# KrishnaswamyLab/MELD

Hardware: AMD Instinct MI355X
Metric: cells/sec through MELD.fit_transform (kNN+Chebyshev) (higher is better)
Workload: dtype f64

## Files before the change

### include/meld_hip.h

```cpp
#ifndef MELD_HIP_H
#define MELD_HIP_H

#include <stddef.h>
#include <stdint.h>

#ifdef __cplusplus
extern "C" {
#endif

#define MELD_OK 0
#define MELD_ERR_INVALID (-1)
#define MELD_ERR_UNSUPPORTED (-2)
#define MELD_ERR_HIP (-3)

typedef void* meld_stream_t;

int meld_abi_version(void);
const char* meld_last_error(void);
int meld_device_count(void);


int meld_knn_padded_dim(int d);
int meld_knn_tile_refs(void);
int meld_knn_block_queries(void);
int meld_knn_row_capacity(int ksel);
double meld_knn_error_coef(int d);

int meld_col_sums_f64(const double* X, int64_t N, int d, double* sums, meld_stream_t stream);
size_t meld_col_stats_temp_bytes(int d);
int meld_col_stats_f64(const double* X, int64_t N, int d, double* sums, double* mins, double* maxs, void* temp, size_t temp_bytes,
                       meld_stream_t stream);

int meld_knn_prepare_refs(const double* X, int64_t N, int d, const double* mean, int KP, float* Rt,
                          float* norm2, float* norm2_max, meld_stream_t stream);
int meld_knn_prepare_queries(const double* X, int64_t N, int d, const double* mean, int KP,
                             int64_t q_begin, int64_t q_count, float* Q, meld_stream_t stream);

int meld_knn_topk(const float* Q, const float* Rt, int64_t n_ref, int KP, int64_t q_count, int ksel,
                  int32_t* cand_idx, float* cand_d2, int32_t* cand_cnt, meld_stream_t stream);

int meld_knn16_kblocks(int d);
int meld_knn16_tile_refs(void);
int meld_knn16_split_dims(int d);
int meld_frame_max_dims(void);
int meld_cov_sample_f64(const double* X, int64_t N, int d, const double* mean, int64_t stride, double* cov, meld_stream_t stream);
int meld_rotate_rows_f64(const double* X, int64_t N, int d, const double* mean, const double* At, double* out, meld_stream_t stream);
int meld_knn16_block_queries(void);
int meld_knn16_row_capacity(int ksel);
double meld_knn16_error_coef(int nprod, int d);
double meld_knn16_error_coef_const(int nprod, int d);
double meld_knn16_error_coef_lin(int nprod);
size_t meld_knn16_tile_bytes(int d);
size_t meld_knn16_query_bytes(int d);
int meld_knn16_prepare(const double* X, int64_t N, int d, const double* mean, int64_t q_begin,
                       int64_t q_count, void* Rt16, void* Q16, float* Qn, float* norm2, float* norm2_max,
                       float* scale_info, meld_stream_t stream);
int meld_knn16_prepare_scaled(const double* X, int64_t N, int d, const double* mean, const double* col_min, const double* col_max,
                              int64_t q_begin, int64_t q_count, void* Rt16, void* Q16, float* Qn, float* norm2, float* norm2_max,
                              float* scale_info, meld_stream_t stream);
size_t meld_knn16_bounds_bytes(int64_t n_ref, int64_t q_count);
size_t meld_knn16_bounds_temp_bytes(int64_t n_ref, int d, int64_t q_count);
int meld_knn16_bounds(const double* X, int64_t N, int d, const double* mean, const float* scale_info,
                      const float* norm2_max, const void* Rt16, int64_t q_begin, int64_t q_count,
                      const float* thr_seed, const float* q_norm2 ,
                      int nprod, void* temp, void* lb2, meld_stream_t stream);
int meld_knn16_tile_spheres(const double* X, int64_t N, int d, const double* mean, const float* scale_info, void* temp,
                            int64_t tile_begin, int64_t tile_count, meld_stream_t stream);
int meld_knn16_sphere_layout(int64_t n_ref, int d, int64_t* rows, int64_t* row_bytes);
int meld_knn16_bounds_from_spheres(const double* X, int64_t N, int d, const double* mean, const float* scale_info,
                      const float* norm2_max, const void* Rt16, int64_t q_begin, int64_t q_count,
                      const float* thr_seed, const float* q_norm2 ,
                      int nprod, void* temp, void* lb2, meld_stream_t stream);
int meld_knn16_prepare_cross(const double* X, int64_t n_refs, int64_t n_total, int d, const double* mean, int64_t q_begin,
                             int64_t q_count, void* Rt16, void* Q16, float* Qn, float* norm2, float* norm2_max,
                             float* scale_info, meld_stream_t stream);
int meld_knn16_prepare_rows(const double* X, int64_t N, int d, const double* mean, const float* scale_info,
                            int64_t q_begin, const int32_t* rows, int64_t n_rows, void* Q16, float* Qn,
                            meld_stream_t stream);
int meld_knn16_research_thresholds(const int32_t* rows, int64_t n_rows, int64_t q_begin, const int32_t* cand_cnt,
// ... 235 lines not shown
```

### meld_amd/_lib.py

```python
from __future__ import annotations

from ._options import is_set, opt

import ctypes as C
import os

_HERE = os.path.dirname(os.path.abspath(__file__))
LIB_NAME = "libmeld_hip.so"
LIB_PATH = os.path.join(_HERE, LIB_NAME)

_i32, _i64, _f64, _sz, _ptr = C.c_int, C.c_int64, C.c_double, C.c_size_t, C.c_void_p

SIGNATURES = {
    "meld_abi_version": (_i32, []),
    "meld_last_error": (C.c_char_p, []),
    "meld_device_count": (_i32, []),
    "meld_knn_padded_dim": (_i32, [_i32]),
    "meld_knn_tile_refs": (_i32, []),
    "meld_knn_block_queries": (_i32, []),
    "meld_knn_row_capacity": (_i32, [_i32]),
    "meld_col_sums_f64": (_i32, [_ptr, _i64, _i32, _ptr, _ptr]),
    "meld_col_stats_temp_bytes": (_sz, [_i32]),
    "meld_col_stats_f64": (_i32, [_ptr, _i64, _i32, _ptr, _ptr, _ptr, _ptr, _sz, _ptr]),
    "meld_knn_prepare_refs": (_i32, [_ptr, _i64, _i32, _ptr, _i32, _ptr, _ptr, _ptr, _ptr]),
# ... 72 lines not shown
        [_ptr, _ptr, _ptr, _ptr, _i64, _i64, _i32, _ptr, _i64, _ptr, _ptr, _ptr, _f64, _f64, _f64, _f64, _ptr, _ptr],
    ),
    "meld_lanczos_steps": (_i32, [_ptr, _ptr, _ptr, _ptr, _i64, _i64, _ptr, _ptr, _ptr, _ptr, _ptr, _ptr, _i32, _i32, _ptr, _ptr]),
    "meld_lanczos_spmv": (_i32, [_ptr, _ptr, _ptr, _ptr, _i64, _i64, _ptr, _i64, _ptr, _ptr, _ptr, _ptr, _ptr]),
    "meld_lanczos_alpha": (_i32, [_ptr, _ptr, _ptr, _ptr, _i32, _ptr]),
    "meld_lanczos_axpy": (_i32, [_ptr, _ptr, _i64, _ptr, _ptr, _ptr]),
    "meld_lanczos_beta": (_i32, [_ptr, _ptr, _ptr, _ptr, _i32, _ptr]),
    "meld_lanczos_fold": (_i32, [_ptr, _ptr, _ptr, _ptr, _i32, _ptr]),
    "meld_lanczos_axpy3": (_i32, [_ptr, _ptr, _ptr, _i64, _ptr, _ptr, _ptr]),
    "meld_pt_geometry": (_i32, [_ptr, _ptr, _ptr, _ptr]),
    "meld_pt_num_blocks": (_i32, [_i64]),
    "meld_pt_seg_len": (_i64, [_i32]),
    "meld_pt_debug_ablate": (_i32, [_i32]),
    "meld_pt_debug_stamps": (_i32, [_ptr]),
    "meld_pt_stream_len": (_i64, [_i64, _i32]),
    "meld_pt_desc_len": (_i64, [_i32]),
    "meld_pt_build": (_i32, [_ptr, _ptr, _ptr, _i64, _i64, _i64, _i32, _ptr, _ptr, _ptr, _ptr]),
    "meld_cheby_step_wide": (_i32, [_ptr, _ptr, _ptr, _ptr, _i64, _i32, _ptr, _i64, _ptr, _ptr, _f64, _f64, _f64, _ptr]),
    "meld_pt_cheby_step": (_i32, [_ptr, _ptr, _ptr, _i64, _i32, _ptr, _i64, _ptr, _ptr, _ptr, _f64, _f64, _f64, _f64, _ptr, _ptr]),
    "meld_pt_cheby_run": (_i32, [_ptr, _ptr, _ptr, _i64, _i32, _ptr, _ptr, _ptr, _ptr, _i32, _f64, _f64, _ptr, _ptr]),
    "meld_pt_lanczos_steps": (_i32, [_ptr, _ptr, _ptr, _i64, _ptr, _ptr, _ptr, _ptr, _ptr, _ptr, _i32, _i32, _ptr, _ptr, _ptr]),
    "meld_pt_lanczos_spmv": (_i32, [_ptr, _ptr, _ptr, _i64, _ptr, _i64, _ptr, _ptr, _ptr, _ptr, _ptr]),
    "meld_kmeans_max_blocks": (_i32, []),
    "meld_kmeans_assign": (_i32, [_ptr, _i64, _i32, _ptr, _i32, _ptr, _ptr, _ptr, _ptr, _i32, _ptr]),
    "meld_scale_f64": (_i32, [_ptr, _f64, _ptr, _i64, _ptr]),
    "meld_axpby_f64": (_i32, [_f64, _ptr, _f64, _ptr, _i64, _ptr, _ptr]),
    "meld_normalize_rows_l1": (_i32, [_ptr, _ptr, _i64, _i32, _ptr]),
    "meld_assign_nearest": (_i32, [_ptr, _i64, _i32, _ptr, _i32, _ptr, _ptr, _ptr, _ptr]),
    "meld_chain_order": (_i32, [_ptr, _i64, _i32, _i32, _ptr, _ptr]),
    "meld_gather_rows_f64": (_i32, [_ptr, _ptr, _i64, _i32, _ptr, _ptr]),
    "meld_frame_max_dims": (_i32, []),
    "meld_cov_sample_f64": (_i32, [_ptr, _i64, _i32, _ptr, _i64, _ptr, _ptr]),
    "meld_rotate_rows_f64": (_i32, [_ptr, _i64, _i32, _ptr, _ptr, _ptr, _ptr]),
    "meld_argsort_u32_temp_bytes": (_sz, [_i64]),
    "meld_argsort_u32": (_i32, [_ptr, _i64, _i32, _ptr, _ptr, _ptr, _sz, _ptr]),
    "meld_order_starts": (_i32, [_ptr, _i64, _i32, _ptr, _ptr]),
    "meld_order_pick_centroids": (_i32, [_ptr, _i64, _i32, _ptr, _ptr, _i32, _i32, _ptr, _ptr]),
    "meld_order_update_keys": (_i32, [_ptr, _ptr, _ptr, _i64, _i32, _ptr]),
    "meld_rccl_available": (_i32, []),
    "meld_rccl_unique_id": (_i32, [_ptr]),
    "meld_rccl_comm_create": (_i32, [_ptr, _i32, _i32, _ptr]),
    "meld_rccl_comm_destroy": (_i32, [_ptr]),
    "meld_rccl_all_gather": (_i32, [_ptr, _ptr, _ptr, _sz, _ptr]),
    "meld_rccl_all_reduce_sum_f64": (_i32, [_ptr, _ptr, _sz, _ptr]),
    "meld_cheby_run_sharded": (_i32, [_ptr, _ptr, _ptr, _ptr, _ptr, _ptr, _i64, _i64, _i64, _i64, _i32, _ptr, _ptr, _ptr, _ptr, _i32, _f64, _f64, _ptr, _ptr]),
    "meld_lanczos_steps_sharded": (_i32, [_ptr, _ptr, _ptr, _ptr, _ptr, _ptr, _i64, _i64, _i64, _i64, _ptr, _ptr, _ptr, _ptr, _ptr, _ptr, _ptr, _i32, _i32, _ptr]),
    "meld_factorize_max_groups": (_i32, []),
    "meld_factorize_max_words": (_i32, []),
    "meld_factorize_temp_bytes": (_sz, [_i64]),
    "meld_factorize_labels": (_i32, [_ptr, _i64, _i32, _ptr, _sz, _ptr, _ptr]),
    "meld_factorize_codes": (_i32, [_ptr, _i64, _ptr, _ptr, _ptr]),
    "meld_indicator_signal": (_i32, [_ptr, _ptr, _ptr, _i64, _i64, _i32, _ptr, _ptr]),
    "meld_scatter_rows_f64": (_i32, [_ptr, _ptr, _i64, _i32, _ptr, _ptr]),
}



class PtLayout(C.Structure):

    _fields_ = [("blk_row", _ptr), ("blk_ntile", _ptr), ("blk_ndist", _ptr), ("seg", _ptr), ("list_cols", _ptr),
                ("pval", _ptr), ("pidx", _ptr), ("nb", C.c_int32), ("pval32", _ptr), ("stream_len", C.c_int64), ("cdesc", _ptr)]


_lib = None


# ... 33 lines not shown
```

### meld_amd/csrc/common.hpp

```cpp
#pragma once
#include <hip/hip_runtime.h>
#include <stdint.h>
#include <stdio.h>
#include <stdlib.h>
#include <string.h>

#include "../../include/meld_hip.h"

namespace meld {

char* err_buf();
void set_err(const char* fmt, ...);

static inline hipStream_t S(meld_stream_t s) { return reinterpret_cast<hipStream_t>(s); }

constexpr int WAVE = 64;

#define MELD_CHECK_ARG(cond, ...)        \
  do {                                   \
    if (!(cond)) {                       \
      meld::set_err(__VA_ARGS__);        \
      return MELD_ERR_INVALID;           \
    }                                    \
  } while (0)

#define MELD_LAUNCH_CHECK(name)                                               \
  do {                                                                        \
    hipError_t e__ = hipGetLastError();                                       \
    if (e__ != hipSuccess) {                                                  \
      meld::set_err("%s: launch failed: %s", name, hipGetErrorString(e__));   \
      return MELD_ERR_HIP;                                                    \
    }                                                                         \
  } while (0)

#define MELD_HIP_CALL(expr)                                                   \
  do {                                                                        \
    hipError_t e__ = (expr);                                                  \
    if (e__ != hipSuccess) {                                                  \
      meld::set_err("%s failed: %s", #expr, hipGetErrorString(e__));          \
      return MELD_ERR_HIP;                                                    \
    }                                                                         \
  } while (0)

__device__ __forceinline__ double wave_sum(double v) {
#pragma unroll
  for (int off = 32; off > 0; off >>= 1) v += __shfl_xor(v, off, 64);
  return v;
}

__device__ __forceinline__ int lane_id() { return threadIdx.x & 63; }

static inline int64_t ceil_div(int64_t a, int64_t b) { return (a + b - 1) / b; }

static inline const char* meld_dev_getenv(const char* name) {
  const char* dev = getenv("MELD_DEV");
  return (dev && dev[0] == '1' && dev[1] == 0) ? getenv(name) : nullptr;
}

struct PtLanczos {
  const double* nrm2_prev;
  double* nrm2_zero;
  const double* state_prev;
  double* state_cur;
  double* betas;
  int it;
  const int* stop;
};

int pt_step(const meld_pt_layout_t* L, const int64_t* rowptr, const double* dw, int p, const double* x_full,
            int64_t x_row_offset, const double* z, double* y, double* r, double alpha, double beta, double gamma,
            double coef, double* dots, const double* coef_dev, hipStream_t st, double coef_x = 0.0, const PtLanczos* lz = nullptr);

}
```

### meld_amd/csrc/frame.hip

```cpp
#include "common.hpp"

namespace meld {

constexpr int FR_ROWS = 64;
constexpr int FR_DMAX = 64;

__global__ __launch_bounds__(256) void cov_sample_kernel(const double* __restrict__ X, int64_t n_s, int64_t stride, int d,
                                                         const double* __restrict__ mean, double* __restrict__ out) {
  __shared__ double sx[FR_ROWS][FR_DMAX + 1];
  const int tid = threadIdx.x;
  const int64_t s0 = (int64_t)blockIdx.x * FR_ROWS;
  const int cnt = (int)min((int64_t)FR_ROWS, n_s - s0);
  for (int u = tid; u < FR_ROWS * d; u += 256) {
    const int r = u / d, k = u - r * d;
    sx[r][k] = r < cnt ? X[(s0 + r) * stride * d + k] - mean[k] : 0.0;
  }
  __syncthreads();
  for (int p = tid; p < d * d; p += 256) {
    const int i = p / d, j = p - i * d;
    if (j < i) continue;
    double acc = 0.0;
    for (int r = 0; r < FR_ROWS; ++r) acc = fma(sx[r][i], sx[r][j], acc);
    atomicAdd(out + p, acc);
  }
}

typedef double f64x8 __attribute__((ext_vector_type(8)));
typedef const __attribute__((address_space(4))) f64x8* const_f64x8_ptr;
constexpr int FR_LD = FR_DMAX + 1;
constexpr int FR_NQ = FR_ROWS * FR_DMAX / 256;
constexpr int FR_CPG = FR_DMAX / 4;
__global__ __launch_bounds__(256) void rotate_rows_kernel(const double* __restrict__ X, int64_t N, int d, const double* __restrict__ mean,
                                                          const double* __restrict__ At, double* __restrict__ out, int64_t tiles_per_wg) {
  __shared__ double sx[FR_ROWS][FR_LD];
  const int tid = threadIdx.x, lane = tid & 63;
  const int w = __builtin_amdgcn_readfirstlane(tid >> 6);
  const int cpg = (d + 3) >> 2;
  const int j0 = w * cpg;
  const int k8n = (d + 7) >> 3;
  const double mk = (lane < d) ? mean[lane] : 0.0;
  const int64_t n_tiles = (N + FR_ROWS - 1) / FR_ROWS;
  const int64_t t_begin = (int64_t)blockIdx.x * tiles_per_wg, t_end = min(n_tiles, t_begin + tiles_per_wg);
// ... 29 lines not shown
        const_f64x8_ptr arow[4];
#pragma unroll
        for (int i = 0; i < 4; ++i)
          arow[i] = (const_f64x8_ptr)(uintptr_t)(At + (size_t)min(j0 + c4 + i, d - 1) * FR_DMAX);
#pragma unroll
        for (int k8 = 0; k8 < FR_DMAX / 8; ++k8) {
          if (k8 < k8n) {
            f64x8 av[4];
#pragma unroll
            for (int i = 0; i < 4; ++i) av[i] = arow[i][k8];
#pragma unroll
            for (int e = 0; e < 8; ++e)
#pragma unroll
              for (int i = 0; i < 4; ++i) acc[i] = fma(xr[8 * k8 + e], av[i][e], acc[i]);
          }
        }
      }
#pragma unroll
      for (int i = 0; i < 4; ++i) res[c4 + i] = acc[i];
    }
    __syncthreads();
#pragma unroll
    for (int c = 0; c < FR_CPG; ++c)
      if (c < cpg && j0 + c < d) sx[lane][j0 + c] = res[c];
    __syncthreads();
#pragma unroll
    for (int q = 0; q < FR_NQ; ++q) {
      const int u = tid + 256 * q, rr = u >> 6, k = u & 63;
      if (rr < cnt && k < d) out[(row0 + rr) * d + k] = sx[rr][k];
    }
  }
}

}

using namespace meld;

extern "C" int meld_frame_max_dims(void) { return FR_DMAX; }

extern "C" int meld_cov_sample_f64(const double* X, int64_t N, int d, const double* mean, int64_t stride, double* cov, meld_stream_t stream) {
  MELD_CHECK_ARG(X && mean && cov && N > 0 && d > 0 && d <= FR_DMAX && stride >= 1, "meld_cov_sample_f64: bad arguments (d <= %d)", FR_DMAX);
  const int64_t n_s = (N + stride - 1) / stride;
  hipLaunchKernelGGL(cov_sample_kernel, dim3((unsigned)ceil_div(n_s, FR_ROWS)), dim3(256), 0, S(stream), X, n_s, stride, d, mean, cov);
  MELD_LAUNCH_CHECK("cov_sample_kernel");
  return MELD_OK;
}

extern "C" int meld_rotate_rows_f64(const double* X, int64_t N, int d, const double* mean, const double* At, double* out, meld_stream_t stream) {
  MELD_CHECK_ARG(X && mean && At && out && N > 0 && d > 0 && d <= FR_DMAX && X != out, "meld_rotate_rows_f64: bad arguments (d <= %d)", FR_DMAX);
  const int64_t tiles = ceil_div(N, FR_ROWS);
  const int64_t per = ceil_div(tiles, (int64_t)1024);
  hipLaunchKernelGGL(rotate_rows_kernel, dim3((unsigned)ceil_div(tiles, per)), dim3(256), 0, S(stream), X, N, d, mean, At, out, per);
  MELD_LAUNCH_CHECK("rotate_rows_kernel");
  return MELD_OK;
}
```

### meld_amd/csrc/knn.hip

```cpp
#include "common.hpp"

#include <algorithm>

namespace meld {

constexpr int KNN_TS = 64;
constexpr int KNN_BQ = 128;
constexpr int KNN_THREADS = 256;
constexpr int KNN_SLACK = 64;
constexpr int KNN_CAPMAX = 192;
constexpr float KNN_BIG = 1.0e30f;

typedef float f32x16 __attribute__((ext_vector_type(16)));

__device__ __forceinline__ float ld_l2_f(const float* p) {
  return __hip_atomic_load(p, __ATOMIC_RELAXED, __HIP_MEMORY_SCOPE_AGENT);
}
__device__ __forceinline__ int ld_l2_i(const int* p) {
  return __hip_atomic_load(p, __ATOMIC_RELAXED, __HIP_MEMORY_SCOPE_AGENT);
}

__device__ float knn_compact_row(int n, int ksel, float* __restrict__ d2row, int* __restrict__ idxrow,
                                 float* sd, int* si, int lane) {
  asm volatile("s_waitcnt vmcnt(0)" ::: "memory");
// ... 256 lines not shown
  float* dst = Q + (size_t)q * KP;
  for (int c = 0; c < KP; ++c)
    dst[c] = (c < d) ? (float)(xrow[c] - mean[c]) : (c == d ? n : (c == d + 1 ? 1.0f : 0.0f));
}

static const int kSupportedKP[] = {8, 12, 16, 24, 32, 40, 52, 64, 80, 104, 128};

}

using namespace meld;

extern "C" int meld_knn_padded_dim(int d) {
  if (d < 1) return MELD_ERR_INVALID;
  for (int kp : kSupportedKP)
    if (d + 2 <= kp) return kp;
  set_err("meld_knn_padded_dim: d=%d exceeds the largest instantiated distance kernel (d <= 126)", d);
  return MELD_ERR_UNSUPPORTED;
}
extern "C" double meld_knn_error_coef(int d) {
  const int kp = meld_knn_padded_dim(d);
  return kp < 0 ? -1.0 : (double)kp * 4.76837158203125e-07;
}
extern "C" int meld_knn_tile_refs(void) { return KNN_TS; }
extern "C" int meld_knn_block_queries(void) { return KNN_BQ; }
extern "C" int meld_knn_row_capacity(int ksel) {
  if (ksel < 1 || ksel > KNN_CAPMAX - KNN_SLACK) {
    set_err("meld_knn_row_capacity: ksel=%d outside [1, %d]", ksel, KNN_CAPMAX - KNN_SLACK);
    return MELD_ERR_UNSUPPORTED;
  }
  return ksel + KNN_SLACK;
}

namespace meld {
constexpr int COL_STATS_GRID = 1024;
__global__ __launch_bounds__(256) void col_stats_kernel(const double* __restrict__ X, int64_t N, int d, double* __restrict__ part) {
  __shared__ double ps[256], pmin[256], pmax[256];
  const int tid = threadIdx.x;
  const int rpp = 256 / d;
  const int c = tid % d;
  const int rl = tid / d;
  double s = 0.0, mn = INFINITY, mx = -INFINITY;
  if (rl < rpp) {
    for (int64_t row = (int64_t)blockIdx.x * rpp + rl; row < N; row += (int64_t)gridDim.x * rpp) {
      const double v = X[row * d + c];
      s += v;
      mn = fmin(mn, v);
      mx = fmax(mx, v);
    }
  }
  ps[tid] = s;
  pmin[tid] = mn;
  pmax[tid] = mx;
  __syncthreads();
  if (tid < d) {
    double ts = 0.0, tmn = INFINITY, tmx = -INFINITY;
    for (int k = 0; k < rpp; ++k) {
      ts += ps[k * d + tid];
      tmn = fmin(tmn, pmin[k * d + tid]);
      tmx = fmax(tmx, pmax[k * d + tid]);
    }
    const size_t g = gridDim.x;
    part[(0 * g + blockIdx.x) * d + tid] = ts;
    part[(1 * g + blockIdx.x) * d + tid] = tmn;
    part[(2 * g + blockIdx.x) * d + tid] = tmx;
  }
}
__global__ __launch_bounds__(256) void col_stats_finish_kernel(const double* __restrict__ part, int grid, int d, double* __restrict__ sums,
                                                               double* __restrict__ mins, double* __restrict__ maxs) {
  __shared__ double ps[256], pmin[256], pmax[256];
  const int c = blockIdx.x, tid = threadIdx.x;
  double ts = 0.0, tmn = INFINITY, tmx = -INFINITY;
  for (int b = tid; b < grid; b += 256) {
    ts += part[((size_t)0 * grid + b) * d + c];
    tmn = fmin(tmn, part[((size_t)1 * grid + b) * d + c]);
    tmx = fmax(tmx, part[((size_t)2 * grid + b) * d + c]);
  }
  ps[tid] = ts;
  pmin[tid] = tmn;
  pmax[tid] = tmx;
  __syncthreads();
  for (int w = 128; w > 0; w >>= 1) {
    if (tid < w) {
      ps[tid] += ps[tid + w];
      pmin[tid] = fmin(pmin[tid], pmin[tid + w]);
      pmax[tid] = fmax(pmax[tid], pmax[tid + w]);
    }
    __syncthreads();
  }
  if (tid == 0) {
    sums[c] = ps[0];
    mins[c] = pmin[0];
    maxs[c] = pmax[0];
  }
}
}
extern "C" size_t meld_col_stats_temp_bytes(int d) { return sizeof(double) * 3 * (size_t)meld::COL_STATS_GRID * (size_t)(d > 0 ? d : 1); }
extern "C" int meld_col_stats_f64(const double* X, int64_t N, int d, double* sums, double* mins, double* maxs, void* temp, size_t temp_bytes,
                                  meld_stream_t stream) {
  using namespace meld;
  MELD_CHECK_ARG(X && sums && mins && maxs && temp && N > 0 && d > 0 && d <= 256, "meld_col_stats_f64: bad arguments (d must be <= 256)");
  MELD_CHECK_ARG(temp_bytes >= meld_col_stats_temp_bytes(d), "meld_col_stats_f64: temp too small");
  const int rpp = 256 / d;
  const int grid = (int)std::min<int64_t>(COL_STATS_GRID, ceil_div(N, rpp));
  hipLaunchKernelGGL(col_stats_kernel, dim3(grid), dim3(256), 0, S(stream), X, N, d, reinterpret_cast<double*>(temp));
  hipLaunchKernelGGL(col_stats_finish_kernel, dim3((unsigned)d), dim3(256), 0, S(stream), reinterpret_cast<const double*>(temp), grid, d,
                     sums, mins, maxs);
  MELD_LAUNCH_CHECK("col_stats_kernel");
  return MELD_OK;
}

extern "C" int meld_col_sums_f64(const double* X, int64_t N, int d, double* sums, meld_stream_t stream) {
  MELD_CHECK_ARG(X && sums && N > 0 && d > 0 && d <= 256, "meld_col_sums_f64: bad arguments (d must be <= 256)");
  MELD_HIP_CALL(hipMemsetAsync(sums, 0, sizeof(double) * d, S(stream)));
  const int rpp = 256 / d;
  int grid = (int)std::min<int64_t>(1024, ceil_div(N, rpp));
  hipLaunchKernelGGL(col_sums_kernel, dim3(grid), dim3(256), 0, S(stream), X, N, d, sums);
  MELD_LAUNCH_CHECK("col_sums_kernel");
  return MELD_OK;
}

extern "C" int meld_knn_prepare_refs(const double* X, int64_t N, int d, const double* mean, int KP, float* Rt,
                                     float* norm2, float* norm2_max, meld_stream_t stream) {
  MELD_CHECK_ARG(X && mean && Rt && norm2 && norm2_max && N > 0, "meld_knn_prepare_refs: null/empty argument");
  MELD_CHECK_ARG(KP == meld_knn_padded_dim(d), "meld_knn_prepare_refs: KP=%d does not match d=%d", KP, d);
  const int64_t n_pad = ceil_div(N, KNN_TS) * KNN_TS;
  hipLaunchKernelGGL(prepare_refs_kernel, dim3((unsigned)ceil_div(n_pad, 256)), dim3(256), 0, S(stream), X, N, d,
// ... 51 lines not shown
```

### meld_amd/graph.py

```python
from __future__ import annotations

from ._options import is_set, opt

import math
import os
import sys
import time

import numpy as np
import torch

from ._lib import check, get_lib, ptr

__all__ = ["DeviceGraph", "build_knn_graph", "default_ksel", "EVENTS", "record_events"]

EVENTS = {"enabled": False, "pairs": []}


def record_events(enabled=True):
    EVENTS["enabled"] = bool(enabled)
    EVENTS["pairs"] = []


class _EventSpan:
# ... 325 lines not shown

            _BLAS_CTL = ThreadpoolController()
        with _BLAS_CTL.limit(limits=1, user_api="blas"):
            return np.linalg.eigh(a, UPLO="U")
    except ImportError:
        return np.linalg.eigh(a, UPLO="U")


def _scan_i32(lib, x, st):
    n = x.shape[0]
    out = torch.empty(n + 1, dtype=torch.int64, device=x.device)
    tb = lib.meld_scan_temp_bytes(n)
    tmp = torch.empty(tb, dtype=torch.uint8, device=x.device)
    check(lib.meld_exclusive_scan_i32_i64(ptr(x), ptr(out), n, ptr(tmp), tb, st), "meld_exclusive_scan_i32_i64")
    return out


class HipOps:

    name = "hip"

    def __init__(self, device=None, search=None, prune=None, nprod=None, spmm=None):
        self.lib = get_lib()
        self.spmm = spmm
        self.nprod = int(opt("MELD_KNN_NPROD", "1")) if nprod is None else int(nprod)
        self.prune = (opt("MELD_KNN_PRUNE", "1") != "0") if prune is None else bool(prune)
        self.radius_cut = opt("MELD_KNN_RADIUS_CUT", "1") != "0"
        self.seed = opt("MELD_KNN_SEED", "1") != "0"
        self.seeded_bounds = opt("MELD_KNN_SEEDED_BOUNDS", "1") != "0"
        self.block_order = opt("MELD_KNN_BLOCK_ORDER", "1") != "0"
        self.step_lists = opt("MELD_KNN_STEP_LISTS", "1") != "0"
        self.rotate = opt("MELD_KNN_ROTATE", "1") != "0"
        self.rotate_min_cells = int(opt("MELD_KNN_ROTATE_MIN", "262144"))
        self.search = search or opt("MELD_KNN_SEARCH", "f16x3")
        if self.search not in ("f16x3", "f32"):
            raise ValueError("unknown search kernel {!r}".format(self.search))
        if not torch.cuda.is_available():
            raise RuntimeError("meld_amd needs a ROCm GPU (MI355X); there is no CPU fallback")
        self.device = torch.device("cuda", torch.cuda.current_device()) if device is None else torch.device(device)

    def col_stats(self, X):
        N, d = int(X.shape[0]), int(X.shape[1])
        out = torch.empty(3, d, dtype=torch.float64, device=X.device)
        tb = self.lib.meld_col_stats_temp_bytes(d)
        tmp = torch.empty(tb, dtype=torch.uint8, device=X.device)
        check(self.lib.meld_col_stats_f64(ptr(X), N, d, ptr(out[0]), ptr(out[1]), ptr(out[2]), ptr(tmp), tb, _stream()), "meld_col_stats_f64")
        return out[0], out[1], out[2]

    def frame_axes_async(self, X, col_stats):
        lib = self.lib
        N, d = int(X.shape[0]), int(X.shape[1])
        if (col_stats is None or opt("MELD_FRAME_ASYNC", "1") == "0" or not self.rotate or not self.prune or not self.step_lists or not self.seed or self.nprod != 1 or self.search != "f16x3"
                or N < max(16384, self.rotate_min_cells) or d > int(lib.meld_frame_max_dims()) or int(lib.meld_knn16_split_dims(d)) <= 0):
            return None
        st = _stream()
        mean = col_stats[0] / N
        cov = torch.zeros(d, d, dtype=torch.float64, device=X.device)
        check(lib.meld_cov_sample_f64(ptr(X), N, d, ptr(mean), max(1, N // 32768), ptr(cov), st), "meld_cov_sample_f64")
        host = torch.empty(d, d, dtype=torch.float64, pin_memory=True)
        host.copy_(cov, non_blocking=True)
        done = torch.cuda.Event()
        done.record()

        def finish(lead):
            done.synchronize()
            evals, evecs = _eigh_one_thread(host.numpy())
            tot = float(evals.sum())
            if not np.isfinite(tot) or tot <= 0.0 or float(evals[-lead:].sum()) < 0.5 * tot:
                return False
            At = np.zeros((d, int(lib.meld_frame_max_dims())))
            At[:, :d] = evecs[:, ::-1].T
            return torch.from_numpy(At).to(X.device, non_blocking=True)

        return finish

    def principal_frame(self, X, mean, lead, comm=None, axes=None):
        lib, st = self.lib, _stream()
        N, d = int(X.shape[0]), int(X.shape[1])
        if axes is not None and (comm is None or getattr(comm, "world", 1) == 1):
            At = axes(lead)
            if At is False:
                return None
            out = torch.empty_like(X)
            check(lib.meld_rotate_rows_f64(ptr(X), N, d, ptr(mean), ptr(At), ptr(out), st), "meld_rotate_rows_f64")
            return out
        wide = d > int(lib.meld_frame_max_dims())
        stride = max(1, N // 32768)
        if wide:
            Xs = X[::stride] - mean
            cov = torch.triu(Xs.T @ Xs)
            del Xs
        else:
            cov = torch.zeros(d, d, dtype=torch.float64, device=X.device)
            check(lib.meld_cov_sample_f64(ptr(X), N, d, ptr(mean), stride, ptr(cov), st), "meld_cov_sample_f64")
        if comm is not None and getattr(comm, "world", 1) > 1:
            if comm.rank != 0:
                cov.zero_()
            comm.all_reduce_sum(cov)
        evals, evecs = _eigh_one_thread(cov.cpu().numpy())
        tot = float(evals.sum())
        if not np.isfinite(tot) or tot <= 0.0 or float(evals[-lead:].sum()) < 0.5 * tot:
            return None
        if wide:
            V = torch.from_numpy(np.ascontiguousarray(evecs[:, ::-1])).to(X.device)
            return torch.addmm(-(mean @ V), X, V)
        At = np.zeros((d, int(lib.meld_frame_max_dims())))
        At[:, :d] = evecs[:, ::-1].T
        At = torch.from_numpy(At).to(X.device)
        out = torch.empty_like(X)
        check(lib.meld_rotate_rows_f64(ptr(X), N, d, ptr(mean), ptr(At), ptr(out), st), "meld_rotate_rows_f64")
        return out

    def directed_kernel_coo(self, X, q_begin, q_count, knn, decay, thresh, ksel, tm=None, force_fallback=False, n_refs=None, assemble=False, comm=None,
                            bw_scale=1.0, bw_fixed=None, col_stats=None, knn_max=None, symm=(0, 0.0), count_rows_ge=None, frame_axes=None):
        lib, st, dev = self.lib, _stream(), X.device
        tm = tm or _Timer(False)
        N, d = int(X.shape[0]), int(X.shape[1])
        cross = n_refs is not None
        NR = int(n_refs) if cross else N
        if cross and not (0 < NR <= q_begin and q_begin + q_count <= N):
            raise ValueError("cross search: the queries must lie behind the n_refs references")
        tm.start()
        col_min = col_max = None
        if col_stats is not None:
            sums, col_min, col_max = col_stats
            mean = sums / N
        elif d <= 256:
            sums, col_min, col_max = self.col_stats(X)
            mean = sums / N
        else:
            mean = X.mean(dim=0)
        norm2 = torch.empty(N, dtype=torch.float32, device=dev)
        nmax = torch.zeros(1, dtype=torch.float32, device=dev)
        X_search, mean_search = X, mean
        search = self.search
        cand_thr, rfac, tiles_done = None, 1.0, None
        used_prune = used_seed = used_seeded_bounds = used_block_order = used_step_lists = used_two_phase = False
        partial_in_search = 0
        if search == "f16x3" and lib.meld_knn16_kblocks(d) < 0:
            search = "wide"
        if cross and search != "f16x3":
            raise NotImplementedError("the search between two point sets runs on the split-fp16 MFMA kernel only (d <= 141)")
        if search == "wide":
            research = None
# ... 16 lines not shown
                    nq = n2[q_begin + q0 : q_begin + q1]
                    best_d = torch.full((q1 - q0, 0), 0.0, dtype=torch.float64, device=dev)
                    best_i = torch.zeros((q1 - q0, 0), dtype=torch.int64, device=dev)
                    for r0 in range(0, N, RC):
                        r1 = min(N, r0 + RC)
                        D = nq[:, None] + n2[None, r0:r1] - 2.0 * (Xq @ Xc[r0:r1].T)
                        ids = torch.arange(r0, r1, device=dev, dtype=torch.int64)[None, :].expand(q1 - q0, -1)
                        D = torch.cat([best_d, D], dim=1)
                        ids = torch.cat([best_i, ids], dim=1)
                        best_d, sel = torch.topk(D, min(kk, D.shape[1]), dim=1, largest=False, sorted=True)
                        best_i = torch.gather(ids, 1, sel)
                    rows = torch.arange(q0, q1, device=dev, dtype=torch.int64)[:, None] * cap + torch.arange(kk, device=dev)[None, :]
                    cand_d2[rows.reshape(-1)] = best_d.clamp_(min=0.0).to(torch.float32).reshape(-1)
                    cand_idx[rows.reshape(-1)] = best_i.to(torch.int32).reshape(-1)
            KP = d
            Q = Rt = None
            del Xc
        elif search == "f16x3":
            nprod = 3 if (self.nprod == 1 and d <= 6) else self.nprod
            KB = lib.meld_knn16_kblocks(d)
            if KB < 0:
                check(KB, "meld_knn16_kblocks")
            TS, BQ = lib.meld_knn16_tile_refs(), lib.meld_knn16_block_queries()
            cap = lib.meld_knn16_row_capacity(ksel)
            if cap < 0:
                check(cap, "meld_knn16_row_capacity")
            err_coef = lib.meld_knn16_error_coef_const(nprod, d)
            err_lin = lib.meld_knn16_error_coef_lin(nprod)
            n_tiles = (NR + TS - 1) // TS
            q_pad = ((q_count + BQ - 1) // BQ) * BQ
            lead = int(lib.meld_knn16_split_dims(d))
            if (self.rotate and lead > 0 and nprod == 1 and not cross and self.prune and self.step_lists and self.seed
                    and N >= max(16384, self.rotate_min_cells) and q_begin % BQ == 0 and bw_fixed is None):
                X_s = self.principal_frame(X, mean, lead, comm, axes=frame_axes)
                if X_s is not None:
                    sums_s, col_min, col_max = self.col_stats(X_s)
                    X_search, mean_search = X_s, sums_s / N
            Rt = torch.empty(n_tiles * lib.meld_knn16_tile_bytes(d), dtype=torch.uint8, device=dev)
            Q = torch.empty(q_pad * lib.meld_knn16_query_bytes(d), dtype=torch.uint8, device=dev)
            Qn = torch.empty(q_pad, dtype=torch.float32, device=dev)
            scale_info = torch.empty(4, dtype=torch.float32, device=dev)
            if cross:
                check(lib.meld_knn16_prepare_cross(ptr(X), NR, N, d, ptr(mean), q_begin, q_count, ptr(Rt), ptr(Q), ptr(Qn), ptr(norm2), ptr(nmax), ptr(scale_info), st), "meld_knn16_prepare_cross")
                norm2[q_begin : q_begin + q_count] = Qn[:q_count]
                nmax = torch.maximum(nmax, Qn[:q_count].max().reshape(1))
            else:
                if col_min is not None:
                    check(lib.meld_knn16_prepare_scaled(ptr(X_search), N, d, ptr(mean_search), ptr(col_min), ptr(col_max), q_begin, q_count, ptr(Rt), ptr(Q), ptr(Qn), ptr(norm2), ptr(nmax), ptr(scale_info), st), "meld_knn16_prepare_scaled")
                else:
                    check(lib.meld_knn16_prepare(ptr(X_search), N, d, ptr(mean_search), q_begin, q_count, ptr(Rt), ptr(Q), ptr(Qn), ptr(norm2), ptr(nmax), ptr(scale_info), st), "meld_knn16_prepare")
            tm.stop("prepare")
            cand_idx = torch.empty(q_pad * cap, dtype=torch.int32, device=dev)
            cand_d2 = torch.empty(q_pad * cap, dtype=torch.float32, device=dev)
            cand_cnt = torch.empty(q_pad, dtype=torch.int32, device=dev)
            if self.radius_cut and knn < ksel:
                cand_thr = torch.full((q_pad,), float("inf"), dtype=torch.float32, device=dev)
                rfac = 1.0 if math.isinf(decay) else float((-math.log(thresh)) ** (1.0 / decay))
                rfac = max(rfac * float(bw_scale), 1.0)
            lb2 = block_order = step_list = step_cnt = None
            tiles_done = torch.zeros(4, dtype=torch.int64, device=dev)
            will_prune = self.prune and q_begin % TS == 0 and N >= 16384 and not cross
            n_blocks = q_pad // BQ
            seeds = None
            knn_cut = knn
            if bw_fixed is not None and cand_thr is not None:
                knn_cut = 0
                rf_real = 1.0 if math.isinf(decay) else float((-math.log(thresh)) ** (1.0 / decay))
                rad = (bw_fixed[q_begin : q_begin + q_count] * float(bw_scale)).clamp_(min=float(np.finfo(float).eps)) * rf_real
                nmx = nmax.to(torch.float64)
# ... 870 lines not shown
```

Measured before the change: 28.06 million.

## Fuse principal-frame rotation with column stats and widen frame to 128 dims

Adds a tiled rotation kernel that computes the rotated rows and, in the same pass, per-column sum, min and max partials, which a shared finish kernel then reduces. This avoids a second full read of the rotated matrix that the separate column-stats pass needed. It also raises the supported frame width from 64 to 128 dims, so the wider case takes the custom rotation path instead of a torch addmm and may be rotated where it was not before. The cost is a more complex kernel with register and LDS tradeoffs that vary with the template width.

```diff
diff --git a/include/meld_hip.h b/include/meld_hip.h
--- a/include/meld_hip.h
+++ b/include/meld_hip.h
@@ -43,8 +43,11 @@
 int meld_knn16_tile_refs(void);
 int meld_knn16_split_dims(int d);
 int meld_frame_max_dims(void);
+int meld_frame_wide_max_dims(void);
 int meld_cov_sample_f64(const double* X, int64_t N, int d, const double* mean, int64_t stride, double* cov, meld_stream_t stream);
 int meld_rotate_rows_f64(const double* X, int64_t N, int d, const double* mean, const double* At, double* out, meld_stream_t stream);
+int meld_rotate_rows_wide_f64(const double* X, int64_t N, int d, const double* mean, const double* At, double* out, double* sums,
+                              double* mins, double* maxs, void* temp, size_t temp_bytes, meld_stream_t stream);
 int meld_knn16_block_queries(void);
 int meld_knn16_row_capacity(int ksel);
 double meld_knn16_error_coef(int nprod, int d);
diff --git a/meld_amd/_lib.py b/meld_amd/_lib.py
--- a/meld_amd/_lib.py
+++ b/meld_amd/_lib.py
@@ -128,6 +128,8 @@
     "meld_frame_max_dims": (_i32, []),
     "meld_cov_sample_f64": (_i32, [_ptr, _i64, _i32, _ptr, _i64, _ptr, _ptr]),
     "meld_rotate_rows_f64": (_i32, [_ptr, _i64, _i32, _ptr, _ptr, _ptr, _ptr]),
+    "meld_frame_wide_max_dims": (_i32, []),
+    "meld_rotate_rows_wide_f64": (_i32, [_ptr, _i64, _i32, _ptr, _ptr, _ptr, _ptr, _ptr, _ptr, _ptr, _sz, _ptr]),
     "meld_argsort_u32_temp_bytes": (_sz, [_i64]),
     "meld_argsort_u32": (_i32, [_ptr, _i64, _i32, _ptr, _ptr, _ptr, _sz, _ptr]),
     "meld_order_starts": (_i32, [_ptr, _i64, _i32, _ptr, _ptr]),
diff --git a/meld_amd/csrc/common.hpp b/meld_amd/csrc/common.hpp
--- a/meld_amd/csrc/common.hpp
+++ b/meld_amd/csrc/common.hpp
@@ -52,6 +52,9 @@
 
 static inline int64_t ceil_div(int64_t a, int64_t b) { return (a + b - 1) / b; }
 
+constexpr int COL_STATS_GRID = 1024;
+int launch_col_stats_finish(const double* part, int grid, int d, double* sums, double* mins, double* maxs, hipStream_t stream);
+
 static inline const char* meld_dev_getenv(const char* name) {
   const char* dev = getenv("MELD_DEV");
   return (dev && dev[0] == '1' && dev[1] == 0) ? getenv(name) : nullptr;
diff --git a/meld_amd/csrc/frame.hip b/meld_amd/csrc/frame.hip
--- a/meld_amd/csrc/frame.hip
+++ b/meld_amd/csrc/frame.hip
@@ -5,9 +5,12 @@
 constexpr int FR_ROWS = 64;
 constexpr int FR_DMAX = 64;
 
+constexpr int FR_WIDE_DMAX = 128;
+
+template <int DMAX>
 __global__ __launch_bounds__(256) void cov_sample_kernel(const double* __restrict__ X, int64_t n_s, int64_t stride, int d,
                                                          const double* __restrict__ mean, double* __restrict__ out) {
-  __shared__ double sx[FR_ROWS][FR_DMAX + 1];
+  __shared__ double sx[FR_ROWS][DMAX + 1];
   const int tid = threadIdx.x;
   const int64_t s0 = (int64_t)blockIdx.x * FR_ROWS;
   const int cnt = (int)min((int64_t)FR_ROWS, n_s - s0);
@@ -103,6 +106,137 @@
   }
 }
 
+
+template <int DP>
+struct RotWide {
+  static constexpr int CPT = DP / 16;
+  static constexpr bool MREG = 256 % DP == 0;
+  static constexpr int NMEAN = MREG ? 0 : DP;
+  static constexpr int RPT = DP * DP + 64 * (DP + 1) + NMEAN <= 20480 ? 4 : 2;
+  static constexpr int RT = 16 * RPT;
+  static constexpr int XLD = RPT == 4 ? DP + 1 : DP;
+  static constexpr int NQ = RT * DP / 256;
+  static_assert(DP * DP + RT * XLD + NMEAN <= 20480, "LDS");
+};
+
+template <int DP>
+__global__ __launch_bounds__(256) void rotate_wide_kernel(const double* __restrict__ X, int64_t N, int d, const double* __restrict__ mean,
+                                                          const double* __restrict__ At, double* __restrict__ out, int64_t tiles_per_wg,
+                                                          double* __restrict__ part) {
+  using G = RotWide<DP>;
+  constexpr int CPT = G::CPT, RPT = G::RPT, RT = G::RT, XLD = G::XLD, NQ = G::NQ;
+  __shared__ double sAt[DP][DP];
+  __shared__ double sX[RT * XLD + G::NMEAN];
+  double* smean = sX + RT * XLD;
+  const int tid = threadIdx.x, tr = tid >> 4, tc = tid & 15;
+  for (int u = tid; u < DP * DP; u += 256) {
+    const int k = u / DP, c = u - k * DP;
+    sAt[k][c] = (k < d && c < d) ? At[(size_t)c * d + k] : 0.0;
+  }
+  double mk = 0.0;
+  if constexpr (G::MREG) {
+    if (tid % DP < d) mk = mean[tid % DP];
+  } else {
+    if (tid < DP) smean[tid] = tid < d ? mean[tid] : 0.0;
+  }
+  const int64_t n_tiles = (N + RT - 1) / RT;
+  const int64_t t_begin = (int64_t)blockIdx.x * tiles_per_wg, t_end = min(n_tiles, t_begin + tiles_per_wg);
+  double xv[NQ];
+  auto fetch = [&](int64_t t) __attribute__((always_inline)) {
+    const int64_t row0 = t * RT;
+#pragma unroll
+    for (int q = 0; q < NQ; ++q) {
+      const int u = tid + 256 * q, rr = u / DP, k = u - rr * DP;
+      xv[q] = (t < t_end && row0 + rr < N && k < d) ? X[(row0 + rr) * d + k] : 0.0;
+    }
+  };
+  double cs[CPT], cmin[CPT], cmax[CPT];
+#pragma unroll
+  for (int j = 0; j < CPT; ++j) cs[j] = 0.0, cmin[j] = INFINITY, cmax[j] = -INFINITY;
+  fetch(t_begin);
+  for (int64_t t = t_begin; t < t_end; ++t) {
+    const int64_t row0 = t * RT;
+    const int cnt = (int)min((int64_t)RT, N - row0);
+    __syncthreads();
+#pragma unroll
+    for (int q = 0; q < NQ; ++q) {
+      const int u = tid + 256 * q, rr = u / DP, k = u - rr * DP;
+      sX[rr * XLD + k] = (rr < cnt && k < d) ? xv[q] - (G::MREG ? mk : smean[k]) : 0.0;
+    }
+    fetch(t + 1);
+    __syncthreads();
+    double acc[RPT][CPT];
+#pragma unroll
+    for (int i = 0; i < RPT; ++i)
+#pragma unroll
+      for (int j = 0; j < CPT; ++j) acc[i][j] = 0.0;
+#pragma unroll 2
+    for (int k = 0; k < d; ++k) {
+      double a[CPT], x[RPT];
+#pragma unroll
+      for (int j = 0; j < CPT; ++j) a[j] = sAt[k][tc + 16 * j];
+#pragma unroll
+      for (int i = 0; i < RPT; ++i) x[i] = sX[(tr + 16 * i) * XLD + k];
+#pragma unroll
+      for (int i = 0; i < RPT; ++i)
+#pragma unroll
+        for (int j = 0; j < CPT; ++j) acc[i][j] = fma(x[i], a[j], acc[i][j]);
+    }
+#pragma unroll
+    for (int i = 0; i < RPT; ++i)
+      if (tr + 16 * i < cnt) {
+#pragma unroll
+        for (int j = 0; j < CPT; ++j) {
+          cs[j] += acc[i][j];
+          cmin[j] = fmin(cmin[j], acc[i][j]);
+          cmax[j] = fmax(cmax[j], acc[i][j]);
+        }
+      }
+    __syncthreads();
+#pragma unroll
+    for (int i = 0; i < RPT; ++i)
+#pragma unroll
+      for (int j = 0; j < CPT; ++j) sX[(tr + 16 * i) * XLD + tc + 16 * j] = acc[i][j];
+    __syncthreads();
+#pragma unroll
+    for (int q = 0; q < NQ; ++q) {
+      const int u = tid + 256 * q, rr = u / DP, k = u - rr * DP;
+      if (rr < cnt && k < d) out[(row0 + rr) * d + k] = sX[rr * XLD + k];
+    }
+  }
+  double* red = DP >= 48 ? &sAt[0][0] : sX;
+  __syncthreads();
+#pragma unroll
+  for (int j = 0; j < CPT; ++j) {
+    red[(0 * 16 + tr) * DP + tc + 16 * j] = cs[j];
+    red[(1 * 16 + tr) * DP + tc + 16 * j] = cmin[j];
+    red[(2 * 16 + tr) * DP + tc + 16 * j] = cmax[j];
+  }
+  __syncthreads();
+  for (int c = tid; c < d; c += 256) {
+    double s = 0.0, mn = INFINITY, mx = -INFINITY;
+    for (int r = 0; r < 16; ++r) {
+      s += red[(0 * 16 + r) * DP + c];
+      mn = fmin(mn, red[(1 * 16 + r) * DP + c]);
+      mx = fmax(mx, red[(2 * 16 + r) * DP + c]);
+    }
+    const size_t g = gridDim.x;
+    part[(0 * g + blockIdx.x) * d + c] = s;
+    part[(1 * g + blockIdx.x) * d + c] = mn;
+    part[(2 * g + blockIdx.x) * d + c] = mx;
+  }
+}
+
+template <int DP>
+static int launch_rotate_wide(const double* X, int64_t N, int d, const double* mean, const double* At, double* out, double* sums, double* mins,
+                              double* maxs, double* part, hipStream_t st) {
+  const int64_t tiles = ceil_div(N, RotWide<DP>::RT);
+  const int64_t per = ceil_div(tiles, (int64_t)COL_STATS_GRID);
+  const int grid = (int)ceil_div(tiles, per);
+  hipLaunchKernelGGL(rotate_wide_kernel<DP>, dim3((unsigned)grid), dim3(256), 0, st, X, N, d, mean, At, out, per, part);
+  MELD_LAUNCH_CHECK("rotate_wide_kernel");
+  return launch_col_stats_finish(part, grid, d, sums, mins, maxs, st);
+}
 }
 
 using namespace meld;
@@ -110,9 +244,12 @@
 extern "C" int meld_frame_max_dims(void) { return FR_DMAX; }
 
 extern "C" int meld_cov_sample_f64(const double* X, int64_t N, int d, const double* mean, int64_t stride, double* cov, meld_stream_t stream) {
-  MELD_CHECK_ARG(X && mean && cov && N > 0 && d > 0 && d <= FR_DMAX && stride >= 1, "meld_cov_sample_f64: bad arguments (d <= %d)", FR_DMAX);
+  MELD_CHECK_ARG(X && mean && cov && N > 0 && d > 0 && d <= FR_WIDE_DMAX && stride >= 1, "meld_cov_sample_f64: bad arguments (d <= %d)", FR_WIDE_DMAX);
   const int64_t n_s = (N + stride - 1) / stride;
-  hipLaunchKernelGGL(cov_sample_kernel, dim3((unsigned)ceil_div(n_s, FR_ROWS)), dim3(256), 0, S(stream), X, n_s, stride, d, mean, cov);
+  if (d <= FR_DMAX)
+    hipLaunchKernelGGL(cov_sample_kernel<FR_DMAX>, dim3((unsigned)ceil_div(n_s, FR_ROWS)), dim3(256), 0, S(stream), X, n_s, stride, d, mean, cov);
+  else
+    hipLaunchKernelGGL(cov_sample_kernel<FR_WIDE_DMAX>, dim3((unsigned)ceil_div(n_s, FR_ROWS)), dim3(256), 0, S(stream), X, n_s, stride, d, mean, cov);
   MELD_LAUNCH_CHECK("cov_sample_kernel");
   return MELD_OK;
 }
@@ -125,3 +262,24 @@
   MELD_LAUNCH_CHECK("rotate_rows_kernel");
   return MELD_OK;
 }
+
+extern "C" int meld_frame_wide_max_dims(void) { return FR_WIDE_DMAX; }
+
+extern "C" int meld_rotate_rows_wide_f64(const double* X, int64_t N, int d, const double* mean, const double* At, double* out, double* sums,
+                                         double* mins, double* maxs, void* temp, size_t temp_bytes, meld_stream_t stream) {
+  MELD_CHECK_ARG(X && mean && At && out && sums && mins && maxs && temp && N > 0 && d > 0 && d <= FR_WIDE_DMAX && X != out,
+                 "meld_rotate_rows_wide_f64: bad arguments (d <= %d)", FR_WIDE_DMAX);
+  MELD_CHECK_ARG(temp_bytes >= meld_col_stats_temp_bytes(d), "meld_rotate_rows_wide_f64: temp too small");
+  double* part = reinterpret_cast<double*>(temp);
+  const hipStream_t st = S(stream);
+  switch ((d + 15) / 16) {
+    case 1: return launch_rotate_wide<16>(X, N, d, mean, At, out, sums, mins, maxs, part, st);
+    case 2: return launch_rotate_wide<32>(X, N, d, mean, At, out, sums, mins, maxs, part, st);
+    case 3: return launch_rotate_wide<48>(X, N, d, mean, At, out, sums, mins, maxs, part, st);
+    case 4: return launch_rotate_wide<64>(X, N, d, mean, At, out, sums, mins, maxs, part, st);
+    case 5: return launch_rotate_wide<80>(X, N, d, mean, At, out, sums, mins, maxs, part, st);
+    case 6: return launch_rotate_wide<96>(X, N, d, mean, At, out, sums, mins, maxs, part, st);
+    case 7: return launch_rotate_wide<112>(X, N, d, mean, At, out, sums, mins, maxs, part, st);
+    default: return launch_rotate_wide<128>(X, N, d, mean, At, out, sums, mins, maxs, part, st);
+  }
+}
diff --git a/meld_amd/csrc/knn.hip b/meld_amd/csrc/knn.hip
--- a/meld_amd/csrc/knn.hip
+++ b/meld_amd/csrc/knn.hip
@@ -312,7 +312,6 @@
 }
 
 namespace meld {
-constexpr int COL_STATS_GRID = 1024;
 __global__ __launch_bounds__(256) void col_stats_kernel(const double* __restrict__ X, int64_t N, int d, double* __restrict__ part) {
   __shared__ double ps[256], pmin[256], pmax[256];
   const int tid = threadIdx.x;
@@ -372,6 +371,11 @@
     mins[c] = pmin[0];
     maxs[c] = pmax[0];
   }
+}
+int launch_col_stats_finish(const double* part, int grid, int d, double* sums, double* mins, double* maxs, hipStream_t stream) {
+  hipLaunchKernelGGL(col_stats_finish_kernel, dim3((unsigned)d), dim3(256), 0, stream, part, grid, d, sums, mins, maxs);
+  MELD_LAUNCH_CHECK("col_stats_finish_kernel");
+  return MELD_OK;
 }
 }
 extern "C" size_t meld_col_stats_temp_bytes(int d) { return sizeof(double) * 3 * (size_t)meld::COL_STATS_GRID * (size_t)(d > 0 ? d : 1); }
diff --git a/meld_amd/graph.py b/meld_amd/graph.py
--- a/meld_amd/graph.py
+++ b/meld_amd/graph.py
@@ -381,6 +381,7 @@
         self.step_lists = opt("MELD_KNN_STEP_LISTS", "1") != "0"
         self.rotate = opt("MELD_KNN_ROTATE", "1") != "0"
         self.rotate_min_cells = int(opt("MELD_KNN_ROTATE_MIN", "262144"))
+        self.fused_prep = opt("MELD_KNN_FUSED_PREP", "1") != "0"
         self.search = search or opt("MELD_KNN_SEARCH", "f16x3")
         if self.search not in ("f16x3", "f32"):
             raise ValueError("unknown search kernel {!r}".format(self.search))
@@ -396,11 +397,34 @@
         check(self.lib.meld_col_stats_f64(ptr(X), N, d, ptr(out[0]), ptr(out[1]), ptr(out[2]), ptr(tmp), tb, _stream()), "meld_col_stats_f64")
         return out[0], out[1], out[2]
 
+    def _frame_dims(self):
+        return int(self.lib.meld_frame_wide_max_dims() if self.fused_prep else self.lib.meld_frame_max_dims())
+
+    def _frame_axes(self, evecs, device):
+        d = evecs.shape[0]
+        At = np.zeros((d, d if self.fused_prep else int(self.lib.meld_frame_max_dims())))
+        At[:, :d] = evecs[:, ::-1].T
+        return torch.from_numpy(At).to(device, non_blocking=True)
+
+    def _rotate(self, X, mean, At):
+        lib, st = self.lib, _stream()
+        N, d = int(X.shape[0]), int(X.shape[1])
+        out = torch.empty_like(X)
+        if not self.fused_prep:
+            check(lib.meld_rotate_rows_f64(ptr(X), N, d, ptr(mean), ptr(At), ptr(out), st), "meld_rotate_rows_f64")
+            return out, None
+        stats = torch.empty(3, d, dtype=torch.float64, device=X.device)
+        tb = lib.meld_col_stats_temp_bytes(d)
+        tmp = torch.empty(tb, dtype=torch.uint8, device=X.device)
+        check(lib.meld_rotate_rows_wide_f64(ptr(X), N, d, ptr(mean), ptr(At), ptr(out), ptr(stats[0]), ptr(stats[1]), ptr(stats[2]), ptr(tmp), tb, st),
+              "meld_rotate_rows_wide_f64")
+        return out, (stats[0], stats[1], stats[2])
+
     def frame_axes_async(self, X, col_stats):
         lib = self.lib
         N, d = int(X.shape[0]), int(X.shape[1])
         if (col_stats is None or opt("MELD_FRAME_ASYNC", "1") == "0" or not self.rotate or not self.prune or not self.step_lists or not self.seed or self.nprod != 1 or self.search != "f16x3"
-                or N < max(16384, self.rotate_min_cells) or d > int(lib.meld_frame_max_dims()) or int(lib.meld_knn16_split_dims(d)) <= 0):
+                or N < max(16384, self.rotate_min_cells) or d > self._frame_dims() or int(lib.meld_knn16_split_dims(d)) <= 0):
             return None
         st = _stream()
         mean = col_stats[0] / N
@@ -417,23 +441,20 @@
             tot = float(evals.sum())
             if not np.isfinite(tot) or tot <= 0.0 or float(evals[-lead:].sum()) < 0.5 * tot:
                 return False
-            At = np.zeros((d, int(lib.meld_frame_max_dims())))
-            At[:, :d] = evecs[:, ::-1].T
-            return torch.from_numpy(At).to(X.device, non_blocking=True)
+            return self._frame_axes(evecs, X.device)
 
         return finish
 
-    def principal_frame(self, X, mean, lead, comm=None, axes=None):
+    def principal_frame(self, X, mean, lead, comm=None, axes=None, with_stats=False):
         lib, st = self.lib, _stream()
         N, d = int(X.shape[0]), int(X.shape[1])
         if axes is not None and (comm is None or getattr(comm, "world", 1) == 1):
             At = axes(lead)
             if At is False:
                 return None
-            out = torch.empty_like(X)
-            check(lib.meld_rotate_rows_f64(ptr(X), N, d, ptr(mean), ptr(At), ptr(out), st), "meld_rotate_rows_f64")
-            return out
-        wide = d > int(lib.meld_frame_max_dims())
+            out, stats = self._rotate(X, mean, At)
+            return (out, stats) if with_stats else out
+        wide = d > self._frame_dims()
         stride = max(1, N // 32768)
         if wide:
             Xs = X[::stride] - mean
@@ -452,13 +473,10 @@
             return None
         if wide:
             V = torch.from_numpy(np.ascontiguousarray(evecs[:, ::-1])).to(X.device)
-            return torch.addmm(-(mean @ V), X, V)
-        At = np.zeros((d, int(lib.meld_frame_max_dims())))
-        At[:, :d] = evecs[:, ::-1].T
-        At = torch.from_numpy(At).to(X.device)
-        out = torch.empty_like(X)
-        check(lib.meld_rotate_rows_f64(ptr(X), N, d, ptr(mean), ptr(At), ptr(out), st), "meld_rotate_rows_f64")
-        return out
+            out = torch.addmm(-(mean @ V), X, V)
+            return (out, None) if with_stats else out
+        out, stats = self._rotate(X, mean, self._frame_axes(evecs, X.device))
+        return (out, stats) if with_stats else out
 
     def directed_kernel_coo(self, X, q_begin, q_count, knn, decay, thresh, ksel, tm=None, force_fallback=False, n_refs=None, assemble=False, comm=None,
                             bw_scale=1.0, bw_fixed=None, col_stats=None, knn_max=None, symm=(0, 0.0), count_rows_ge=None, frame_axes=None):
@@ -541,9 +559,10 @@
             lead = int(lib.meld_knn16_split_dims(d))
             if (self.rotate and lead > 0 and nprod == 1 and not cross and self.prune and self.step_lists and self.seed
                     and N >= max(16384, self.rotate_min_cells) and q_begin % BQ == 0 and bw_fixed is None):
-                X_s = self.principal_frame(X, mean, lead, comm, axes=frame_axes)
-                if X_s is not None:
-                    sums_s, col_min, col_max = self.col_stats(X_s)
+                framed = self.principal_frame(X, mean, lead, comm, axes=frame_axes, with_stats=True)
+                if framed is not None:
+                    X_s, stats_s = framed
+                    sums_s, col_min, col_max = stats_s if stats_s is not None else self.col_stats(X_s)
                     X_search, mean_search = X_s, sums_s / N
             Rt = torch.empty(n_tiles * lib.meld_knn16_tile_bytes(d), dtype=torch.uint8, device=dev)
             Q = torch.empty(q_pad * lib.meld_knn16_query_bytes(d), dtype=torch.uint8, device=dev)
```

After: 28.41 million (median of 6 runs). No clear change (+1.3%).
